# CommonRoad/commonroad-reactive-planner

Measured on AMD Instinct MI355X. Metric: candidate trajectories/sec (sample+cost+collision) per replan, higher is better.
Workload: dtype f64; 1 GPU; cfg3: DEU_Test-1_1_T-1, 31x31x63 grid, N=60, 51 obstacles (49 synthetic, seed 0); mode=draw, horizon_steps=60, n_obstacles=51, parallelism=one GPU, exchange=none

## Files before the change

### commonroad-reactive-planner_amd/csrc/rp_host.hip

```cpp
#include <hip/hip_runtime.h>
#include <hip/hip_ext.h>
#include <sched.h>

#include <algorithm>
#include <atomic>
#include <chrono>
#include <cmath>
#include <cstdio>
#include <cstdlib>
#include <cstring>
#include <mutex>
#include <new>
#include <string>
#include <unordered_map>
#include <vector>

#include "rp_kernels.h"
#include "rp_frontend.h"
#include "rp_corridor.h"
#include "rp_pool.h"

namespace {

constexpr int kBlocksPerCU = 4;
constexpr int kFoldPartials = 256;
constexpr int kFoldThreshold = 8192;
constexpr size_t kAutoMaterializeBytes = 64u << 20;
constexpr size_t kLdsTableLimit = 65536;
constexpr int kChunkMinWavesPerCU = 7;
constexpr int kCostMinPerCU = 832;
constexpr int kSweepMinPerCU = 512;
constexpr int kLazyCap[RP_LAZY_LEVELS] = {1024, 4096, 16384};
constexpr int kLazyOff[RP_LAZY_LEVELS] = {0, 1024, 5120};
constexpr int kLazyListWords = 21504;
constexpr uint32_t kLazyTarget[RP_LAZY_LEVELS] = {128, 1024, 8192};

using ResultBlock = FinalizeOut;

struct Options {
    int lanes = 0;
    int eval_block = 0;
    int cost_kernel = -1;
    int chunk_kernel = -1;
    int lazy = -1;
    int sweep = -1;
    int fused_lon = 1;
    int fused_lon_blocks = -1;
    int auto_materialize = 1;
    int stage_out = 1, row_padding = 1, row_align = 0, tail_split = 1;
    int table_window = 1;
    int fold_threshold = kFoldThreshold;
    int lon_publish = 1, inline_grids = 1, event_bracket = 0, winner_lanes_as_batch = 0, zero_copy = 1, coeff_groups = 1;
    int winner_skip_query = 1;
    int lazy_trace = 0, print_stamps = 0, timing = 0;
    int wait_mode = RP_WAIT_SPIN;
};
struct OptionDesc {
    const char *key;
    int Options::*field;
    const char *env;
    bool env_negates;
    int lo, hi;
};
const OptionDesc kOptionTable[] = {
    {"lanes", &Options::lanes, "RP_AMD_G", false, 0, 64},
    {"eval_block", &Options::eval_block, "RP_AMD_EVAL_BLOCK", false, 0, 256},
    {"cost_kernel", &Options::cost_kernel, "RP_AMD_COST_KERNEL", false, -1, 1},
    {"chunk_kernel", &Options::chunk_kernel, "RP_AMD_CHUNK_KERNEL", false, -1, 1},
    {"lazy", &Options::lazy, "RP_AMD_LAZY", false, -1, 1},
    {"sweep", &Options::sweep, "RP_AMD_SWEEP", false, -1, 1},
    {"fused_lon", &Options::fused_lon, "RP_AMD_NO_FUSED_LON", true, 0, 1},
    {"fused_lon_blocks", &Options::fused_lon_blocks, "RP_AMD_FUSED_LON_BLOCKS", false, -1, 1 << 20},
    {"auto_materialize", &Options::auto_materialize, "RP_AMD_NO_AUTO_MATERIALIZE", true, 0, 1},
    {"stage_out", &Options::stage_out, "RP_AMD_NO_STAGE_OUT", true, 0, 1},
    {"row_padding", &Options::row_padding, "RP_AMD_NO_ROW_PADDING", true, 0, 1},
    {"row_align", &Options::row_align, "RP_AMD_ROW_ALIGN", false, 0, 16},
    {"tail_split", &Options::tail_split, "RP_AMD_NO_TAIL_SPLIT", true, 0, 1},
    {"table_window", &Options::table_window, "RP_AMD_NO_TABLE_WINDOW", true, 0, 1},
    {"fold_threshold", &Options::fold_threshold, "RP_AMD_FOLD_THRESHOLD", false, 1, 1 << 30},
    {"lon_publish", &Options::lon_publish, "RP_AMD_NO_LON_PUBLISH", true, 0, 1},
    {"inline_grids", &Options::inline_grids, "RP_AMD_NO_INLINE_GRIDS", true, 0, 1},
    {"event_bracket", &Options::event_bracket, "RP_AMD_EVENT_BRACKET", false, 0, 1},
    {"winner_lanes_as_batch", &Options::winner_lanes_as_batch, "RP_AMD_WINNER_G_AS_BATCH", false, 0, 1},
    {"winner_skip_query", &Options::winner_skip_query, "RP_AMD_NO_WINNER_SKIP_QUERY", true, 0, 1},
    {"zero_copy", &Options::zero_copy, "RP_AMD_NO_ZERO_COPY", true, 0, 1},
    {"coeff_groups", &Options::coeff_groups, "RP_AMD_NO_COEFF_GROUPS", true, 0, 1},
    {"lazy_trace", &Options::lazy_trace, "RP_AMD_LAZY_TRACE", false, 0, 1},
    {"print_stamps", &Options::print_stamps, "RP_AMD_PRINT_STAMPS", false, 0, 1},
    {"timing", &Options::timing, "RP_AMD_TIMING", false, 0, 1},
    {"wait_mode", &Options::wait_mode, "RP_AMD_WAIT_MODE", false, RP_WAIT_SPIN, RP_WAIT_EVENT},
};
const OptionDesc *find_option(const char *key) {
    if (!key) return nullptr;
    for (const OptionDesc &d : kOptionTable)
        if (std::strcmp(d.key, key) == 0) return &d;
    return nullptr;
}
void options_from_environment(Options &o) {
    for (const OptionDesc &d : kOptionTable) {
        const char *e = d.env ? std::getenv(d.env) : nullptr;
        if (!e) continue;
        const int v = d.env_negates ? 0 : std::atoi(e);
        if (v >= d.lo && v <= d.hi) o.*(d.field) = v;
    }
}

}

struct rp_ctx {
    Options opt;
// ... 18 lines not shown
    std::vector<double> h_sobb, h_tri, h_circ;
    std::vector<int32_t> h_clus_info;
    bool grid_valid = false;
    double grid_ego_r = 0.0;
    int32_t *d_clus_info = nullptr;
    ObsTables obs{};

    char *h_stage = nullptr, *d_stage = nullptr;
    size_t cap_stage = 0;
    std::vector<char> staged;
    bool staged_on_device = false;
    uint32_t *d_status = nullptr;
    double *d_cost = nullptr, *d_user = nullptr;
    size_t cap_status = 0, cap_cost = 0, cap_user = 0;
    double *d_states = nullptr;
    double *d_compact = nullptr;
    size_t cap_compact = 0;
    size_t cap_states = 0;
    double *d_profile = nullptr, *d_profile_one = nullptr;
    size_t cap_profile = 0, cap_profile_one = 0;
    PairHdr *d_pair_hdr = nullptr, *d_pair_hdr_one = nullptr;
    size_t cap_pair_hdr = 0;
    void *d_partials = nullptr;
    int cap_partials = 0;
    unsigned long long *d_sel_scratch = nullptr;
    LazyCtl *d_lazy_ctl = nullptr;
    int32_t *d_lazy_lists = nullptr;
    uint32_t *d_lazy_hist = nullptr;
    double *d_lazy_states = nullptr;
    size_t cap_lazy_states = 0;
    int lazy_skip = 0, lazy_penalty = 0;
    int collision_mode = RP_COLLISION_AUTO;
    int last_kernel = 0;
    int last_lazy = 0;
    double last_best_cost = 0.0;
    int64_t last_best_index = -1;
    double path_us[2] = {0.0, 0.0};
    int path_n[2] = {0, 0};
    int path_since_probe = 0, path_regime = -1;
    bool path_adaptive = false;
    bool time_whole = false;
    std::chrono::steady_clock::time_point plan_t0;
    bool epilogue_dirty = false;
    struct Pending {
        bool active = false, cin = false, skip_eval = false, ticket = false, done = false, time_valid = false, mat = false, coeffs = false;
        unsigned long long seq = 0;
        int grid = 0;
        KArgs ka{};
        std::chrono::steady_clock::time_point tp0, tp1;
    } pending;
    struct LevelState {
        Pending pending;
        std::vector<char> staged;
        bool staged_on_device = false, last_rows_on_device = false;
        int last_G = 0, last_block = 0, last_kernel = 0, last_lazy = 0;
        size_t last_fused_lds = 0;
        int grid_index = 0;
    };
    std::vector<LevelState> chain;
    int chain_total = 0;
    unsigned long long *d_gate = nullptr;
    unsigned long long *d_sweep = nullptr;
    struct ChainInputs {
        rp_params p; rp_cost cost; std::vector<rp_grids> grids; std::vector<std::vector<double>> T, L, D; std::vector<std::vector<int32_t>> tl;
        int want = 0;
    } chain_in;
// ... 116 lines not shown
        if (f && hipExtModuleLaunchKernel(f, (uint32_t)grid * (uint32_t)block, 1, 1, (uint32_t)block, 1, 1, lds, c->stream, nullptr, extra,
                                          c->ev0, c->ev1, 0) == hipSuccess) {
            c->timed_by_launch = true;
            return;
        }
        (void)hipGetLastError();
    }
    if (!f || hipModuleLaunchKernel(f, (unsigned)grid, 1, 1, (unsigned)block, 1, 1, (unsigned)lds, c->stream, nullptr, extra) != hipSuccess) {
        (void)hipGetLastError();
        void *args[] = {const_cast<void *>(args_block)};
        (void)hipLaunchKernel(kernel, dim3(grid), dim3(block), args, lds, c->stream);
    }
}

int collision_level(const KArgs &ka) {
    if (!ka.has_obstacles || (ka.flags & RP_FLAG_SKIP_COLLISION)) return 0;
    return (ka.obs.n_sobb + ka.obs.n_tri + ka.obs.n_circ) > 0 ? 2 : 1;
}

const void *sweep_kernel_fn(bool cin, int coll, bool one_chunk) {
    if (cin) {
        if (coll == 2) return one_chunk ? (const void *)rp_eval_kernel<16, false, true, 2, true, false, false, RP_BLOCK, true> : (const void *)rp_eval_kernel<16, false, true, 2, false, false, false, RP_BLOCK, true>;
        return one_chunk ? (const void *)rp_eval_kernel<16, false, true, 1, true, false, false, RP_BLOCK, true> : (const void *)rp_eval_kernel<16, false, true, 1, false, false, false, RP_BLOCK, true>;
    }
    if (coll == 2) return one_chunk ? (const void *)rp_eval_kernel<16, false, false, 2, true, false, false, RP_BLOCK, true> : (const void *)rp_eval_kernel<16, false, false, 2, false, false, false, RP_BLOCK, true>;
    return one_chunk ? (const void *)rp_eval_kernel<16, false, false, 1, true, false, false, RP_BLOCK, true> : (const void *)rp_eval_kernel<16, false, false, 1, false, false, false, RP_BLOCK, true>;
}

const void *chunk_kernel_fn(bool low, int coll) {
    if (low) return coll == 2 ? (const void *)rp_chunk_kernel<true, 2> : (coll == 1 ? (const void *)rp_chunk_kernel<true, 1> : (const void *)rp_chunk_kernel<true, 0>);
    return coll == 2 ? (const void *)rp_chunk_kernel<false, 2> : (coll == 1 ? (const void *)rp_chunk_kernel<false, 1> : (const void *)rp_chunk_kernel<false, 0>);
}

template <int G, bool MAT, bool CIN, int COLL, bool STAGE>
void launch_eval_tcs(rp_ctx *c, const KArgs &ka, int grid, size_t lds, int block = RP_BLOCK) {
    if constexpr (G == 16 && !STAGE) {
        if (block == 64) {
            if (ka.N + 1 <= G) launch_kargs(c, (const void *)rp_eval_kernel<G, MAT, CIN, COLL, true, false, false, 64>, grid, 64, lds, ka);
            else launch_kargs(c, (const void *)rp_eval_kernel<G, MAT, CIN, COLL, false, false, false, 64>, grid, 64, lds, ka);
            return;
        }
    }
    if (ka.N + 1 <= G) launch_kargs(c, (const void *)rp_eval_kernel<G, MAT, CIN, COLL, true, STAGE, false>, grid, RP_BLOCK, lds, ka);
    else launch_kargs(c, (const void *)rp_eval_kernel<G, MAT, CIN, COLL, false, STAGE, false>, grid, RP_BLOCK, lds, ka);
}

constexpr int kFusedLonG = 16;
constexpr size_t kFusedLonLdsLimit = 61440;
int fused_lon_max_blocks(const rp_ctx *c) {
    if (c->opt.fused_lon_blocks >= 0) return c->opt.fused_lon_blocks;
    return c->num_cus * 4;
}

size_t fused_lon_lds(const rp_ctx *c, const KArgs &ka, int64_t count, int G, bool cin, bool mat, int *pairs) {
    if (count <= 0 || !(G == kFusedLonG || (G == 64 && mat && ka.N + 1 <= 64) || (G == 32 && mat && ka.N + 1 <= 32))) return 0;
    const int gpb = RP_BLOCK / G;
    if ((count + gpb - 1) / gpb > (int64_t)fused_lon_max_blocks(c)) return 0;
    const int P = cin ? gpb : std::min<int64_t>(gpb, ((int64_t)gpb + ka.nD - 2) / ka.nD + 1);
    const size_t slot_bytes = ka.has_obstacles ? (size_t)ka.obs.n_clus * ka.obs.clus_per * RP_SLOT_ROW * sizeof(double) : 0;
    const size_t bytes = (size_t)ka.table_words * sizeof(double) + slot_bytes +
                         (size_t)P * ((size_t)PF_STRIDE * (size_t)(ka.N + 1) * sizeof(double) + sizeof(PairHdr) + sizeof(int) + sizeof(double)) + 16;
    if (bytes > kFusedLonLdsLimit) return 0;
    *pairs = P;
    return (bytes + 15) & ~(size_t)15;
}

template <bool MAT, bool CIN, int COLL>
void launch_eval_fused_c(rp_ctx *c, const KArgs &ka, int grid, size_t lds, int lanes) {
// ... 451 lines not shown
            kl.grids_inline = lon_inline ? 1 : 0;
            kl.publish_grids = lon_publish ? 1 : 0;
            launch_lon(c, kl, cin);
        }
        const bool by_launch = timed && count > 0 && !c->opt.event_bracket;
        const int n_steps = ka.N + 1;
        const int chunk_nb = (n_steps + RP_CHUNK_STEPS - 1) / RP_CHUNK_STEPS;
        const int chunk_G = (chunk_nb >= 2 && chunk_nb <= RP_CHUNK_MAX_BLOCKS) ? chunk_nb : 0;
        const bool lane_kernel_ok = count > 0 && !fused_lds && !cin && !(ka.flags & RP_FLAG_DRAW_ALL) && !ka.single_index && !ka.index_list &&
                                    ka.cost_kind != RP_COST_EXTERNAL;
        const bool cost_rows_ok = (unsigned long long)ka.pair_count * PF_FIELDS * (unsigned long long)(ka.N + 1) * 8ull < (1ull << 32);
        const bool cost_big = count >= (int64_t)c->num_cus * 1024;
        auto lane_kernel_for = [&](int coll) -> int {
            if (!lane_kernel_ok) return 0;
            if (c->opt.chunk_kernel == 1 && chunk_G) return 2;
            if (!cost_rows_ok) return (chunk_G && c->opt.chunk_kernel != 0 && coll == 0) ? 2 : 0;
            if (c->opt.cost_kernel == 1) return 1;
            if (coll > 0) return (c->opt.cost_kernel != 0 && cost_big) ? 1 : 0;
            const int64_t chunk_waves = ((count + RP_CHUNK_BLOCK - 1) / RP_CHUNK_BLOCK) * chunk_G;
            const bool chunk_ok = c->opt.chunk_kernel != 0 && chunk_G && chunk_G <= 4 && chunk_waves >= (int64_t)c->num_cus * kChunkMinWavesPerCU;
            if (c->opt.cost_kernel != 0 && count >= (int64_t)c->num_cus * (chunk_ok ? kCostMinPerCU : (ka.N + 1 <= 64 ? 240 : 448))) return 1;
            return chunk_ok ? 2 : 0;
        };
        auto launch_main_eval = [&](const KArgs &k, bool mat_) -> int {
            c->timed_by_launch = false;
            c->time_next_launch = by_launch;
            if (timed && !by_launch) HIP_TRY(c, hipEventRecord(c->ev0, c->stream));
            const auto te0 = c->timing ? std::chrono::steady_clock::now() : std::chrono::steady_clock::time_point();
            const int coll = collision_level(k);
            const int which = mat_ ? 0 : lane_kernel_for(coll);
            if (which == 1) {
                main_grid = (int)((count + RP_COST_BLOCK - 1) / RP_COST_BLOCK);
                c->last_kernel = RP_KERNEL_COST;
                const void *fn = k.low_vel_mode
                    ? (coll == 2 ? (const void *)rp_cost_kernel<true, 2> : coll == 1 ? (const void *)rp_cost_kernel<true, 1> : (const void *)rp_cost_kernel<true, 0>)
                    : (coll == 2 ? (const void *)rp_cost_kernel<false, 2> : coll == 1 ? (const void *)rp_cost_kernel<false, 1> : (const void *)rp_cost_kernel<false, 0>);
                launch_kargs(c, fn, main_grid, RP_COST_BLOCK, 0, k);
            } else if (which == 2) {
                main_grid = (int)((count + RP_CHUNK_BLOCK - 1) / RP_CHUNK_BLOCK);
                c->last_kernel = RP_KERNEL_CHUNK;
                launch_kargs(c, chunk_kernel_fn(k.low_vel_mode != 0, coll), main_grid, RP_CHUNK_BLOCK * chunk_G, rp_chunk_lds_bytes(chunk_G), k);
            } else {
                main_grid = grid;
                c->last_kernel = RP_KERNEL_EVAL;
                if (fused_lds) launch_eval_fused(c, k, grid, mat_, cin, fused_lds, G);
                else launch_eval(c, k, grid, mat_, cin, G, block);
            }
            if (c->timing) c->t_sum[4] += std::chrono::duration<double, std::micro>(std::chrono::steady_clock::now() - te0).count();
            c->time_next_launch = false;
            if (timed && !by_launch) HIP_TRY(c, hipEventRecord(c->ev1, c->stream));
            time_valid = timed && (!by_launch || c->timed_by_launch);
            return RP_OK;
        };
        bool lazy_possible = count > 0 && !mat && !fused_lds && collision_level(ka) > 0 && !(ka.flags & RP_FLAG_DRAW_ALL) &&
                             ka.cost_kind != RP_COST_EXTERNAL && !ka.single_index && !ka.gate;
        const int lazy_env = c->opt.lazy;
        lazy_possible = lazy_possible && lazy_env != 0 && (c->collision_mode != RP_COLLISION_EAGER || lazy_env == 1);
        const bool always = lazy_env == 1 || (lazy_env == -1 && c->collision_mode == RP_COLLISION_COST_ORDERED);
        bool lazy_try = lazy_possible && (always || (!small && c->lazy_skip == 0));
        if (lazy_possible && !lazy_try && !always && !small && c->lazy_skip > 0) --c->lazy_skip;
        c->path_adaptive = lazy_possible && lazy_env == -1 && !small && c->collision_mode == RP_COLLISION_TIMED;
        if (c->path_adaptive) {
            int lg = 0;
            while ((count >> (lg + 1)) != 0) ++lg;
            const int regime = 2 * lg + (cin ? 1 : 0);
            if (regime != c->path_regime) { c->path_regime = regime; c->path_n[0] = c->path_n[1] = 0; c->path_since_probe = 0; }
            if (lazy_try) {
                if (c->path_n[1] == 0) lazy_try = true;
                else if (c->path_n[0] == 0) lazy_try = c->path_n[1] < 4;
                else {
                    lazy_try = c->path_us[1] <= c->path_us[0];
                    if (++c->path_since_probe >= 64) { lazy_try = !lazy_try; c->path_since_probe = 0; }
                }
            }
        }
        c->last_lazy = 0;
        const bool sweep_first = lazy_try && c->opt.sweep == 1 && !fused_lds;
// ... 322 lines not shown
int rp_last_path(const rp_ctx *c) { return c ? c->last_lazy : 0; }
int rp_last_kernel(const rp_ctx *c) { return c ? c->last_kernel : 0; }

int rp_set_collision_path(rp_ctx *c, int mode) {
    if (!c) return RP_EINVAL;
    if (mode < RP_COLLISION_AUTO || mode > RP_COLLISION_TIMED) return fail(c, RP_EINVAL, "rp_set_collision_path: unknown mode");
    if (mode != c->collision_mode) { c->lazy_skip = c->lazy_penalty = 0; c->path_regime = -1; }
    c->collision_mode = mode;
    return RP_OK;
}

int rp_set_profiling(rp_ctx *c, int enable) {
    if (!c) return RP_EINVAL;
    c->profiling = enable < 0 ? 0 : enable;
    return RP_OK;
}

int rp_set_option(rp_ctx *c, const char *key, int64_t value) {
    if (!c) return RP_EINVAL;
    if (c->pending.active) return fail(c, RP_ESTATE, "rp_set_option: a plan is in flight on this context (rp_plan_wait first)");
    const OptionDesc *d = find_option(key);
    if (!d) return fail(c, RP_EINVAL, std::string("rp_set_option: unknown option '") + (key ? key : "(null)") + "'");
    if (value < d->lo || value > d->hi) return fail(c, RP_EINVAL, std::string("rp_set_option: value out of range for '") + key + "'");
    c->opt.*(d->field) = (int)value;
    c->timing = c->opt.timing != 0;
    c->spin_wait = c->opt.wait_mode != RP_WAIT_EVENT;
    c->lazy_skip = c->lazy_penalty = 0; c->path_regime = -1;
    return RP_OK;
}

int rp_get_option(const rp_ctx *c, const char *key, int64_t *value) {
    if (!c || !value) return RP_EINVAL;
    if (key && std::strcmp(key, "wait_fallbacks") == 0) { *value = c->wait_fallbacks; return RP_OK; }
    const OptionDesc *d = find_option(key);
    if (!d) return RP_EINVAL;
    *value = c->opt.*(d->field);
    return RP_OK;
}

int rp_set_wait_mode(rp_ctx *c, int mode) { return rp_set_option(c, "wait_mode", mode); }
int rp_get_wait_mode(const rp_ctx *c) { return c ? c->opt.wait_mode : RP_WAIT_SPIN; }

int rp_set_reference(rp_ctx *c, int32_t n, const double *ref_pos, const double *ref_theta, const double *ref_curv,
                     const double *ref_curv_d, const double *ref_x, const double *ref_y, double proj_domain_d_limit) {
    if (!c) return RP_EINVAL;
    if (c->pending.active) return fail(c, RP_ESTATE, "rp_set_reference: a plan is in flight on this context (rp_plan_wait first)");
    if (n < 2 || !ref_pos || !ref_theta || !ref_curv || !ref_curv_d || !ref_x || !ref_y)
        return fail(c, RP_EINVAL, "rp_set_reference: need n >= 2 and six non-null tables");
    for (int i = 0; i + 1 < n; ++i)
        if (!(ref_pos[i + 1] > ref_pos[i])) return fail(c, RP_EINVAL, "rp_set_reference: ref_pos must be strictly increasing");
    HIP_TRY(c, hipSetDevice(c->device));
    std::vector<double> t((size_t)TB_ROWS * (size_t)n);
    std::memcpy(&t[(size_t)TB_POS * n], ref_pos, sizeof(double) * n);
    std::memcpy(&t[(size_t)TB_THETA * n], ref_theta, sizeof(double) * n);
    std::memcpy(&t[(size_t)TB_CURV * n], ref_curv, sizeof(double) * n);
    std::memcpy(&t[(size_t)TB_CURV_D * n], ref_curv_d, sizeof(double) * n);
    std::memcpy(&t[(size_t)TB_X * n], ref_x, sizeof(double) * n);
    std::memcpy(&t[(size_t)TB_Y * n], ref_y, sizeof(double) * n);
    double *tx = &t[(size_t)TB_TX * n], *ty = &t[(size_t)TB_TY * n];
    std::vector<double> ux(n - 1), uy(n - 1);
    for (int i = 0; i + 1 < n; ++i) {
        double ex = ref_x[i + 1] - ref_x[i], ey = ref_y[i + 1] - ref_y[i];
        double ln = std::sqrt(ex * ex + ey * ey);
        if (!(ln > 0.0)) return fail(c, RP_EINVAL, "rp_set_reference: duplicate polyline vertices");
        ux[i] = ex / ln; uy[i] = ey / ln;
    }
// ... 1256 lines not shown
```

### commonroad-reactive-planner_amd/csrc/rp_kernels.h

```cpp
#pragma once

#include "rp_device.h"

#define RP_BLOCK 256
#ifndef RP_COPY_OUT_STORE
#define RP_COPY_OUT_STORE(p, v)                                                                                   \
    __builtin_nontemporal_store(*reinterpret_cast<const __attribute__((ext_vector_type(2))) double *>(&(v)),        \
                                reinterpret_cast<__attribute__((ext_vector_type(2))) double *>(p))
#endif
#ifndef RP_WAVES_PER_SIMD
#define RP_WAVES_PER_SIMD 3
#endif

struct KArgs {
    double dt;
    int32_t N, factor, time_step0, low_vel_mode, lon_mode;
    uint32_t constraint_mask, flags;
    double x0_lon[3], x0_lat[3], x0_orientation;
    double wheelbase, wb_rear_axle, half_length, half_width, ego_radius;
    double a_max, v_switch, v_delta_max, kappa_max;
    double c_yaw;
    double c_kdot;
    int32_t cost_kind, has_speed, has_s, partials_cap;
    double w_a, desired_speed, desired_d, desired_s;
// ... 832 lines not shown
            for (int l = 0; l < RP_LAZY_LEVELS; ++l) total[l] += (unsigned int)__popcll(__ballot(lvl[u] == l));
        unsigned int at[RP_LAZY_LEVELS] = {0, 0, 0};
#pragma unroll
        for (int l = 0; l < RP_LAZY_LEVELS; ++l)
            if (total[l] && lane == 0) at[l] = atomicAdd(&a.ctl->count[l], total[l]);
#pragma unroll
        for (int l = 0; l < RP_LAZY_LEVELS; ++l) at[l] = (unsigned int)__builtin_amdgcn_readfirstlane((int)at[l]);
#pragma unroll
        for (int u = 0; u < kUnroll; ++u) {
            const int i = base0 + u * RP_GATHER_THREADS + lane;
#pragma unroll
            for (int l = 0; l < RP_LAZY_LEVELS; ++l) {
                const unsigned long long bm = __ballot(lvl[u] == l);
                const unsigned int pos = at[l] + (unsigned int)__popcll(bm & lt_mask);
                if (lvl[u] == l && pos < (unsigned int)a.cap[l]) a.lists[a.off[l] + (int)pos] = (int32_t)(a.cand_begin + i);
                at[l] += (unsigned int)__popcll(bm);
            }
        }
    }
}

__device__ __forceinline__ double frenet_kterm(double k_r_d, double d, double k_r, double dp) { return __builtin_fma(k_r_d, d, k_r * dp); }
__device__ __forceinline__ double frenet_kappa(double dpp, double kterm, double tanT, double cosT, double q, double k_r) {
    return __builtin_fma(k_r, q, (__builtin_fma(kterm, tanT, dpp) * cosT) * (q * q));
}
__device__ __forceinline__ double heading_cos(double cos_ref, double sin_ref, double cosT, double sinT) { return __builtin_fma(cos_ref, cosT, -(sin_ref * sinT)); }
__device__ __forceinline__ double heading_sin(double cos_ref, double sin_ref, double cosT, double sinT) { return __builtin_fma(sin_ref, cosT, cos_ref * sinT); }
__device__ __forceinline__ double frenet_acc(double sdd, double f, double sd, double secT, double oneKrD, double tanT, double kappa, double k_r,
                                             double kterm) {
    return __builtin_fma(sdd, f, (sd * sd * secT) * __builtin_fma(oneKrD * tanT, __builtin_fma(kappa, f, -k_r), -kterm));
}


template <class KA>
__device__ __forceinline__ double cost_terms(const KA &a, int i, int N, int mid, double acc, double v, double s, double d, double th_cl) {
    double e, cst;
    e = a.w_a * acc; cst = e * e;
    e = 0.25 * (a.desired_d - d); cst = __builtin_fma(e, e, cst);
    e = 0.25 * fabs(th_cl); cst = __builtin_fma(e, e, cst);
    if (a.has_speed) { e = 5.0 * (v - a.desired_speed); cst = __builtin_fma(e, e, cst); }
    if (a.has_s) { e = 0.25 * (a.desired_s - s); cst = __builtin_fma(e, e, cst); }
    if (i == N) {
        e = 20.0 * (a.desired_d - d); cst = __builtin_fma(e, e, cst);
        e = 5.0 * fabs(th_cl); cst = __builtin_fma(e, e, cst);
        if (a.has_speed) { e = v - a.desired_speed; cst += 50.0 * (e * e); }
        if (a.has_s) { e = 20.0 * (a.desired_s - s); cst = __builtin_fma(e, e, cst); }
    }
    if (i == mid && a.has_speed) { e = v - a.desired_speed; cst += 100.0 * (e * e); }
    return cst;
}

template <class KA>
__device__ __forceinline__ uint32_t constraint_reason(const KA &a, uint32_t cm, double v, double acc, double kappa, double dth, double kdot) {
    uint32_t reason = RP_REASON_NONE;
    const double a_max = a.a_max, v_switch = a.v_switch, kappa_max = a.kappa_max;
    const double wk = a.wheelbase * kappa;
    const bool bad_yaw = fabs(rint(dth * a.c_yaw)) > kappa_max * v * 1e5;
    const bool bad_kd = fabs(kdot) > a.c_kdot * __builtin_fma(wk, wk, 1.0);
    const bool fast = v > v_switch;
    const double acc_l = fast ? acc * v : acc, acc_r = fast ? a_max * v_switch : a_max;
    const bool bad_acc = !((-a_max <= acc) & (acc_l <= acc_r));
    const bool bad_v = v < -RP_EPS, bad_k = fabs(kappa) > kappa_max;
    reason = (((cm & RP_CHECK_ACCELERATION) != 0) & bad_acc) ? RP_REASON_ACCELERATION : reason;
    reason = (((cm & RP_CHECK_KAPPA_DOT) != 0) & bad_kd) ? RP_REASON_KAPPA_DOT : reason;
    reason = (((cm & RP_CHECK_YAW_RATE) != 0) & bad_yaw) ? RP_REASON_YAW_RATE : reason;
    reason = (((cm & RP_CHECK_KAPPA) != 0) & bad_k) ? RP_REASON_KAPPA : reason;
// ... 513 lines not shown
template <bool COEFFS_IN>
__device__ __forceinline__ void fetch_lateral(const KArgs &a, int64_t gidx, CandIn &ci, int64_t hdr_pair0) {
    int64_t pair;
    if (COEFFS_IN) {
        const double *pt = a.lat_coeffs + 6 * gidx;
#pragma unroll
        for (int k = 0; k < 6; ++k) ci.v[k] = pt[k];
        pair = pair_index<true>(a, gidx);
    } else {
        const uint32_t g32 = (uint32_t)gidx, nd = (uint32_t)a.nD;
        const uint32_t p32 = g32 / nd;
        pair = p32;
        ci.v[0] = grid_base(a)[a.nT + a.nL + (int)(g32 - p32 * nd)];
    }
    ci.pair_slot = pair - hdr_pair0;
}

__device__ __forceinline__ void fetch_header(const PairHdr *hdrs, CandIn &ci) {
    const PairHdr h = hdrs[ci.pair_slot];
    ci.lat_T = h.lat_T;
    ci.s0 = h.s0;
    ci.pre_reason = h.pre_reason;
    ci.L = h.L;
}

template <bool COEFFS_IN>
__device__ __forceinline__ CandIn fetch_candidate(const KArgs &a, int64_t gidx, const PairHdr *hdrs, int64_t hdr_pair0) {
    CandIn ci;
    fetch_lateral<COEFFS_IN>(a, gidx, ci, hdr_pair0);
    fetch_header(hdrs, ci);
    return ci;
}

template <int G, bool MAT, bool COEFFS_IN, int COLL, bool ONE_CHUNK, bool STAGE_OUT, bool LON_FUSED, int BLOCK = RP_BLOCK, bool SWEEP = false>
__global__ __launch_bounds__(BLOCK, RP_WAVES_PER_SIMD) void rp_eval_kernel(const KArgsG ag) {
    static_assert(!SWEEP || (G == 16 && !MAT && COLL != 0 && !STAGE_OUT && !LON_FUSED && BLOCK == RP_BLOCK), "the sweep's variant");
    const KArgs &a = ag.k;
    extern __shared__ double lds_out[];
    static_assert(!(LON_FUSED && STAGE_OUT), "the single-launch variant stores state rows directly");
    constexpr bool RP_WT = LON_FUSED;
    constexpr bool RP_NT = MAT && !LON_FUSED && !STAGE_OUT;
    touch_kernargs<10>();

    const int tid = threadIdx.x;
    RP_STAMP(0);
    RP_TL(0);
    const int lane = tid & 63;
    const int gl = lane & (G - 1);
    const int gbase = lane & ~(G - 1);
    static_assert(BLOCK == RP_BLOCK || (!LON_FUSED && !STAGE_OUT), "smaller workgroups: plain two-kernel variants only");
    constexpr int GPB = BLOCK / G;
    constexpr int GPW = 64 / G;
    constexpr int PFN = COLL ? PF_FIELDS : PF_COS_REF;
    const int wave_in_block = tid >> 6;
    const int group_in_wave = gbase / G;
    const int grp = tid / G;

    if (level_gate_closed(a.gate, a.gate_seq, a.gate_level)) return;
    if (a.single_index && *a.single_index < 0) {
        if (a.host_seq && a.ticket_if_none && tid == 0) __hip_atomic_store(a.host_seq, a.seq_value, __ATOMIC_RELEASE, __HIP_MEMORY_SCOPE_SYSTEM);
        return;
    }
    const int64_t wave_first = ((int64_t)blockIdx.x * GPB) + (int64_t)wave_in_block * GPW;
    int64_t count_ = a.single_index ? 1 : a.count;
    if (!LON_FUSED && a.index_list) {
        const uint32_t lc = *a.list_count;
        count_ = (int64_t)(lc < (uint32_t)a.list_cap ? lc : (uint32_t)a.list_cap);
        if ((int64_t)blockIdx.x * GPB >= count_) {
            if (a.partials) {
// ... 286 lines not shown
    }
    RP_STAMP(1);

    typedef const KArgs __attribute__((address_space(4))) *kargs_cptr;
    kargs_cptr ap_late = (LON_FUSED || MAT) ? (kargs_cptr)__builtin_amdgcn_kernarg_segment_ptr() : (kargs_cptr)&a;
    if (LON_FUSED) asm volatile("" : "+s"(ap_late));
    const KArgs __attribute__((address_space(4))) &al = *ap_late;
    const int N = al.N, n = N + 1;
    const int nchunks = ONE_CHUNK ? 1 : (n + G - 1) / G;
    const double dt = al.dt;
    const bool draw = (al.flags & RP_FLAG_DRAW_ALL) != 0;
    const bool low = al.low_vel_mode != 0;
    const uint32_t cm = al.constraint_mask;
    const int mid = n / 2;
    double *const gs_poly = sh_grp[grp].poly;
    double *const gs_last = sh_grp[grp].last;

    auto eval_cost_terms = [&](int i, double acc, double v, double s, double d, double th_cl) -> double {
        double e, cst;
        e = al.w_a * acc; cst = e * e;
        e = 0.25 * (al.desired_d - d); cst = __builtin_fma(e, e, cst);
        e = 0.25 * fabs(th_cl); cst = __builtin_fma(e, e, cst);
        if (al.has_speed) { e = 5.0 * (v - al.desired_speed); cst = __builtin_fma(e, e, cst); }
        if (al.has_s) { e = 0.25 * (al.desired_s - s); cst = __builtin_fma(e, e, cst); }
        if (i == N) {
            e = 20.0 * (al.desired_d - d); cst = __builtin_fma(e, e, cst);
            e = 5.0 * fabs(th_cl); cst = __builtin_fma(e, e, cst);
            if (al.has_speed) { e = v - al.desired_speed; cst += 50.0 * (e * e); }
            if (al.has_s) { e = 20.0 * (al.desired_s - s); cst = __builtin_fma(e, e, cst); }
        }
        if (i == mid && al.has_speed) { e = v - al.desired_speed; cst += 100.0 * (e * e); }
        return cst;
    };

    if (wave_first < count) {
        const int64_t w0 = wave_first;
        const int64_t slot = w0 + group_in_wave;
        const bool valid = slot < count && sweep_need;
        const int64_t gidx = al.single_index ? *al.single_index
                             : ((!LON_FUSED && al.index_list) ? (int64_t)al.index_list[valid ? slot : w0] : al.cand_begin + (valid ? slot : w0));

        const int L = cin.L;
        const double s0 = cin.s0;
        const uint32_t pre_reason = (uint32_t)cin.pre_reason;
        const int32_t pair_slot_ = (int32_t)(pair_index<COEFFS_IN>(al, gidx) - pair0);
        const int32_t pair_w = __builtin_amdgcn_readfirstlane(pair_slot_);
        const uint32_t n8p = (uint32_t)n * 8u;
        const char *const pbase = reinterpret_cast<const char *>(prof_base + ((size_t)pair_w * PF_FIELDS) * (size_t)n);
        const uint32_t poff8 = (uint32_t)(pair_slot_ - pair_w) * PF_FIELDS * n8p;
        ProfStep pf = pf0;
        if (!LON_FUSED) {
            Poly lat;
            if (COEFFS_IN) lat = {cin.v[0], cin.v[1], cin.v[2], cin.v[3], cin.v[4], cin.v[5]};
            else lat = quintic_coeffs(al.x0_lat[0], al.x0_lat[1], al.x0_lat[2], cin.v[0], 0.0, 0.0, cin.lat_T);
            if (gl == 0) park_poly(gs_poly, lat);
        }
        RP_STAMP(2);

        int fail_step = -1, ood_step = -1;
        uint32_t fail_reason = RP_REASON_NONE;
        bool collide = false;
        double cost_acc = 0.0;

        bool alive = valid && pre_reason == RP_REASON_NONE;
        if (__ballot(alive) != 0) {
            double theta_carry = al.x0_orientation;
            double kappa_carry = 0.0;
            double cumx = 0.0, cumy = 0.0;
            const bool store_ok = MAT && valid && pre_reason == RP_REASON_NONE;
            const int ns = (MAT && !STAGE_OUT) ? al.row_stride : n;
            constexpr bool SPLIT_OK = MAT && !STAGE_OUT && !LON_FUSED && G == 16;
            const int tail_m = SPLIT_OK ? al.tail_split : 0;
            const uint32_t cand8 = (uint32_t)state_block_doubles(ns, tail_m) * 8u;
            char *const obase = !MAT ? nullptr
                                : (STAGE_OUT ? reinterpret_cast<char *>(lds_out + (size_t)(wave_in_block * GPW) * RP_N_ARRAYS * (size_t)n)
                                             : reinterpret_cast<char *>(al.states) + (size_t)w0 * (size_t)cand8);
            const uint32_t n8 = (uint32_t)ns * 8u;
            const uint32_t lane_off8 = (uint32_t)group_in_wave * (STAGE_OUT ? RP_N_ARRAYS * n8 : cand8);
            constexpr bool ROW_MULV = LON_FUSED;
            constexpr bool LATE_STORE = MAT && !STAGE_OUT;
            uint32_t n8v = n8;
            auto row_at = [&](uint32_t off8, int row) -> double * {
                return reinterpret_cast<double *>(obase + (size_t)(ROW_MULV ? __umul24((uint32_t)row, n8v) + off8 : off8 + (uint32_t)row * n8));
            };

#pragma nounroll
            for (int c = 0; c < nchunks; ++c) {
                const int base = c * G;
                const int i = base + gl;
                const bool live = i <= N;
                const bool act = i < L;
                if (ROW_MULV) asm volatile("" : "+v"(n8v));

                if (!ONE_CHUNK && c > 0) {
                    if (LON_FUSED) pf = load_profile_item<PFN>(prof_base + ((size_t)pair_slot_ * (size_t)n + (size_t)(live ? i : N)) * PF_STRIDE);
                    else pf = load_profile<PFN, G == 16>(pbase, poff8 + (uint32_t)(live ? i : N) * 8u, n8p);
                }
                double s = pf.f[PF_S], sd = pf.f[PF_SD], sdd = pf.f[PF_SDD];
                const double inv_sd = pf.f[PF_INV_SD], th_ref = pf.f[PF_TH_REF];
                const double k_r = pf.f[PF_KR], k_r_d = pf.f[PF_KRD];
                const double px = pf.f[PF_PX], py = pf.f[PF_PY], nx = pf.f[PF_NX], ny = pf.f[PF_NY];
                const bool s_in_dom = pf.f[PF_INDOM] != 0.0;

                constexpr bool SKIP_EXTENDED = !(MAT && COLL == 0);
                double d = 0.0, dd = 0.0, ddd = 0.0, th_cl = 0.0, th_gl = 0.0, cos_gl = 1.0, sin_gl = 0.0;
                double kappa = 0.0, v = 0.0, acc = 0.0, kdot = 0.0, x = 0.0, y = 0.0;
                uint64_t near_sta_cell = 0;
                if (!SKIP_EXTENDED || __any(act)) {
                    const double t = (double)i * dt;
                    const double tau = low ? s - s0 : t;
                    d = poly_pos(gs_poly, tau); dd = poly_vel(gs_poly, tau); ddd = poly_acc(gs_poly, tau);
                    if (fabs(dd) < RP_EPS) dd = 0.0;
                    if (!LATE_STORE && store_ok && act) {
                        const uint32_t off8 = lane_off8 + (uint32_t)i * 8u;
                        st_row<RP_WT, RP_NT>(row_at(off8, RP_S), s);
                        st_row<RP_WT, RP_NT>(row_at(off8, RP_S_DOT), sd);
                        st_row<RP_WT, RP_NT>(row_at(off8, RP_S_DDOT), sdd);
                        st_row<RP_WT, RP_NT>(row_at(off8, RP_D), d);
                        st_row<RP_WT, RP_NT>(row_at(off8, RP_D_DOT), dd);
                        st_row<RP_WT, RP_NT>(row_at(off8, RP_D_DDOT), ddd);
                    }
                    RP_STAMP(3);

                    const bool moving = inv_sd > 0.0;
                    double dp, dpp;
                    lateral_derivs(low, dd, ddd, inv_sd, sdd, dp, dpp);

                    const bool use_atan = moving || low;
                    double cosT, secT, tanT;
                    atan_angles(dp, th_ref, th_cl, th_gl, cosT, secT, tanT);
                    if (__any(act && !use_atan)) {
                        const uint64_t mv = group_ballot<G>(use_atan && act, gbase);
                        const uint64_t below = mv & ((1ull << gl) - 1ull);
                        const int src = below ? 63 - __clzll(below) : 0;
                        const double th_from = group_bcast<G>(th_gl, src);
                        if (!use_atan) {
                            th_gl = below ? th_from : theta_carry;
// ... 15 lines not shown
                    RP_STAMP(6);

                    uint32_t reason = constraint_reason(al, cm, v, acc, kappa, dth, kdot);
                    reason = act ? reason : RP_REASON_NONE;
                    if (__any(reason != RP_REASON_NONE)) {
                        const uint64_t fm = group_ballot<G>(reason != RP_REASON_NONE, gbase);
                        const int fl = fm ? __ffsll((unsigned long long)fm) - 1 : 0;
                        const uint32_t r_first = (uint32_t)__shfl((int)reason, fl, G);
                        if (fm && fail_step < 0) { fail_step = base + fl; fail_reason = r_first; }
                        if (!draw && fail_step >= 0) alive = false;
                        if (__ballot(alive) == 0) break;
                    }
                    RP_STAMP(7);

                    const bool in_dom = s_in_dom && fabs(d) <= al.proj_d_limit;
                    x = px + d * nx; y = py + d * ny;
                    if (__any(act && !in_dom) || ood_step >= 0) {
                        const uint64_t om = group_ballot<G>(act && !in_dom, gbase);
                        if (om && ood_step < 0) ood_step = base + __ffsll((unsigned long long)om) - 1;
                        if (ood_step >= 0 && i >= ood_step) { x = 0.0; y = 0.0; }
                    }
                    if (act) {
                        if (!LATE_STORE && store_ok) {
                            const uint32_t off8 = lane_off8 + (uint32_t)i * 8u;
                            st_row<RP_WT, RP_NT>(row_at(off8, RP_X), x);
                            st_row<RP_WT, RP_NT>(row_at(off8, RP_Y), y);
                            st_row<RP_WT, RP_NT>(row_at(off8, RP_THETA), th_gl);
                            st_row<RP_WT, RP_NT>(row_at(off8, RP_V), v);
                            st_row<RP_WT, RP_NT>(row_at(off8, RP_A), acc);
                            st_row<RP_WT, RP_NT>(row_at(off8, RP_KAPPA), kappa);
                            st_row<RP_WT, RP_NT>(row_at(off8, RP_KAPPA_DOT), kdot);
                            st_row<RP_WT, RP_NT>(row_at(off8, RP_THETA_CL), th_cl);
                        }
                        cost_acc += eval_cost_terms(i, acc, v, s, d, th_cl);
                    }
                    if (COLL == 2 && live && alive && fail_step < 0 && ood_step < 0 && !collide && act)
                        near_sta_cell = static_grid_mask(al.obs.grid, al.obs.gx0, al.obs.gy0, al.obs.ginv, al.obs.gnx, al.obs.gny,
                                                         x + al.wb_rear_axle * cos_gl, y + al.wb_rear_axle * sin_gl);
                }
                const bool cell_wanted = COLL == 2 && live && alive && fail_step < 0 && ood_step < 0 && !collide;
                RP_STAMP(8);

                const int ll = L - 1 - base;
                const bool take = (ll >= 0 && ll < G);
                if (__any(take && L < n)) {
                    if (!COLL) rp_sincos(th_gl, &sin_gl, &cos_gl);
                    if (take && gl == ll) {
                        double *o = gs_last;
                        o[0] = x; o[1] = y; o[2] = th_gl; o[3] = v; o[4] = acc; o[5] = kappa; o[6] = kdot;
                        o[7] = s; o[8] = d; o[9] = th_cl; o[10] = sd; o[11] = sdd; o[12] = dd; o[13] = ddd;
                        o[14] = cos_gl; o[15] = sin_gl;
                    }
                }
                if (!ONE_CHUNK && c + 1 < nchunks) {
                    theta_carry = group_bcast<G>(th_gl, G - 1);
                    kappa_carry = group_bcast<G>(kappa, G - 1);
                }
                if (__any(live && !act)) {
                    double termx = 0.0, termy = 0.0;
                    const double *o = gs_last;
                    const double tk = (double)(i - L + 1) * dt;
                    double vt = 0.0;
                    if (!act) {
                        vt = o[3] + tk * o[4];
                        vt = vt * (vt >= 0.0 ? 1.0 : 0.0);
                        termx = dt * vt * o[14];
                        termy = dt * vt * o[15];
                    }
                    const double scx = group_scan<G>(termx) + cumx, scy = group_scan<G>(termy) + cumy;
                    if (!act) {
                        x = o[0] + scx;
                        y = o[1] + scy;
                        th_gl = o[2];
                        cos_gl = o[14];
                        sin_gl = o[15];
                        const double sv = o[10] + tk * 0.0;
                        const double e_sd = sv * (sv >= 0.0 ? 1.0 : 0.0);
                        const double e_dd = o[12] + tk * 0.0;
                        const double e_s = o[7] + tk * o[10];
                        const double e_d = o[8] + tk * o[12];
                        if (live) cost_acc += eval_cost_terms(i, o[4], vt, e_s, e_d, o[9]);
                        if (LATE_STORE) {
                            v = vt; acc = o[4]; kappa = o[5]; kdot = o[6];
                            s = e_s; d = e_d; th_cl = o[9];
                            sd = e_sd; sdd = o[11]; dd = e_dd; ddd = o[13];
                        } else if (store_ok && live) {
                            {
                                const uint32_t off8 = lane_off8 + (uint32_t)i * 8u;
                                st_row<RP_WT, RP_NT>(row_at(off8, RP_X), x);
                                st_row<RP_WT, RP_NT>(row_at(off8, RP_Y), y);
                                st_row<RP_WT, RP_NT>(row_at(off8, RP_THETA), th_gl);
                                st_row<RP_WT, RP_NT>(row_at(off8, RP_V), vt);
                                st_row<RP_WT, RP_NT>(row_at(off8, RP_A), o[4]);
                                st_row<RP_WT, RP_NT>(row_at(off8, RP_KAPPA), o[5]);
                                st_row<RP_WT, RP_NT>(row_at(off8, RP_KAPPA_DOT), o[6]);
                                st_row<RP_WT, RP_NT>(row_at(off8, RP_S), e_s);
                                st_row<RP_WT, RP_NT>(row_at(off8, RP_D), e_d);
                                st_row<RP_WT, RP_NT>(row_at(off8, RP_THETA_CL), o[9]);
                                st_row<RP_WT, RP_NT>(row_at(off8, RP_S_DOT), e_sd);
                                st_row<RP_WT, RP_NT>(row_at(off8, RP_S_DDOT), o[11]);
                                st_row<RP_WT, RP_NT>(row_at(off8, RP_D_DOT), e_dd);
                                st_row<RP_WT, RP_NT>(row_at(off8, RP_D_DDOT), o[13]);
                            }
                        }
                    }
                    if (!ONE_CHUNK && c + 1 < nchunks) {
                        cumx = group_bcast<G>(scx, G - 1);
                        cumy = group_bcast<G>(scy, G - 1);
                    }
                }
                if (COLL == 2) {
                    if (cell_wanted && !act)
                        near_sta_cell = static_grid_mask(al.obs.grid, al.obs.gx0, al.obs.gy0, al.obs.ginv, al.obs.gnx, al.obs.gny,
                                                         x + al.wb_rear_axle * cos_gl, y + al.wb_rear_axle * sin_gl);
                    uint32_t c_lo = (uint32_t)near_sta_cell, c_hi = (uint32_t)(near_sta_cell >> 32);
                    asm volatile("" : "+v"(c_lo), "+v"(c_hi));
                    near_sta_cell = ((uint64_t)c_hi << 32) | c_lo;
                }
                if (SPLIT_OK && tail_m > 0 && base >= tail_m) {
                    if (store_ok) {
                        char *const tbase = obase + (size_t)(lane_off8 + (uint32_t)(RP_N_ARRAYS * tail_m) * 8u + (uint32_t)gl * 8u);
                        const bool lo = gl < 8;
                        auto pair_store = [&](int q, double r0, double r1) {
                            const double up = dpp_f64<DPP_ROW_SHR8, 0xf>(r1);
                            st_row<RP_WT, RP_NT>(reinterpret_cast<double *>(tbase + q * 128), lo ? r0 : up);
                        };
                        pair_store(0, x, y); pair_store(1, th_gl, v); pair_store(2, acc, kappa); pair_store(3, kdot, s);
                        pair_store(4, d, th_cl); pair_store(5, sd, sdd); pair_store(6, dd, ddd);
                    }
                } else
                if (LATE_STORE && store_ok && i < ns) {
                    const uint32_t off8 = lane_off8 + (uint32_t)i * 8u;
                    st_row<RP_WT, RP_NT>(row_at(off8, RP_X), x);
                    st_row<RP_WT, RP_NT>(row_at(off8, RP_Y), y);
                    st_row<RP_WT, RP_NT>(row_at(off8, RP_THETA), th_gl);
                    st_row<RP_WT, RP_NT>(row_at(off8, RP_V), v);
                    st_row<RP_WT, RP_NT>(row_at(off8, RP_A), acc);
                    st_row<RP_WT, RP_NT>(row_at(off8, RP_KAPPA), kappa);
                    st_row<RP_WT, RP_NT>(row_at(off8, RP_KAPPA_DOT), kdot);
                    st_row<RP_WT, RP_NT>(row_at(off8, RP_S), s);
                    st_row<RP_WT, RP_NT>(row_at(off8, RP_D), d);
                    st_row<RP_WT, RP_NT>(row_at(off8, RP_THETA_CL), th_cl);
                    st_row<RP_WT, RP_NT>(row_at(off8, RP_S_DOT), sd);
                    st_row<RP_WT, RP_NT>(row_at(off8, RP_S_DDOT), sdd);
                    st_row<RP_WT, RP_NT>(row_at(off8, RP_D_DOT), dd);
                    st_row<RP_WT, RP_NT>(row_at(off8, RP_D_DDOT), ddd);
                }
                RP_STAMP(9);

                if (COLL) {
                    const bool want = live && alive && fail_step < 0 && ood_step < 0 && !collide;
                    bool hit = false;
                    constexpr bool masked = !COEFFS_IN;
                    const uint64_t near_dyn = double_as_mask(pf.f[PF_NEAR]);
                    const double ego_cx = x + al.wb_rear_axle * cos_gl, ego_cy = y + al.wb_rear_axle * sin_gl;
                    const uint64_t near_sta = want ? near_sta_cell : 0;
                    const bool ask = want && ((!masked && al.obs.n_dyn > 0) || (near_dyn | near_sta) != 0);
                    RP_STAMP(44);
#ifdef RP_WALK_COUNT
                    if (a.debug && !a.single_index && blockIdx.x == RP_STAMP_BLOCK && threadIdx.x == RP_STAMP_THREAD) rp_walk_dbg = a.debug + 40;
#endif
// ... 721 lines not shown
```

Baseline: 455.4 million candidates/s.

## Add fixed 64-stride eval kernel variant with deferred, freshly fetched cost params

Adds a ROW64 template specialization of the eval kernel, used when the row stride is 64, tail split is off and the horizon fits in 64 steps. With a compile-time stride, state-row addresses are computed from a single mid-row base with constant offsets. Cost evaluation and static-grid lookup move out of the inner loop to after the extension, with cost parameters reloaded from a scalar pointer. The intent is to cut address arithmetic and register pressure in the materializing path, at the cost of another kernel instantiation and a different cost-accumulation point.

```diff
diff --git a/commonroad-reactive-planner_amd/csrc/rp_host.hip b/commonroad-reactive-planner_amd/csrc/rp_host.hip
--- a/commonroad-reactive-planner_amd/csrc/rp_host.hip
+++ b/commonroad-reactive-planner_amd/csrc/rp_host.hip
@@ -48,6 +48,7 @@
     int fused_lon_blocks = -1;
     int auto_materialize = 1;
     int stage_out = 1, row_padding = 1, row_align = 0, tail_split = 1;
+    int fixed_stride = 1;
     int table_window = 1;
     int fold_threshold = kFoldThreshold;
     int lon_publish = 1, inline_grids = 1, event_bracket = 0, winner_lanes_as_batch = 0, zero_copy = 1, coeff_groups = 1;
@@ -76,6 +77,7 @@
     {"row_padding", &Options::row_padding, "RP_AMD_NO_ROW_PADDING", true, 0, 1},
     {"row_align", &Options::row_align, "RP_AMD_ROW_ALIGN", false, 0, 16},
     {"tail_split", &Options::tail_split, "RP_AMD_NO_TAIL_SPLIT", true, 0, 1},
+    {"fixed_stride", &Options::fixed_stride, "RP_AMD_NO_FIXED_STRIDE", true, 0, 1},
     {"table_window", &Options::table_window, "RP_AMD_NO_TABLE_WINDOW", true, 0, 1},
     {"fold_threshold", &Options::fold_threshold, "RP_AMD_FOLD_THRESHOLD", false, 1, 1 << 30},
     {"lon_publish", &Options::lon_publish, "RP_AMD_NO_LON_PUBLISH", true, 0, 1},
@@ -160,6 +162,7 @@
     int lazy_skip = 0, lazy_penalty = 0;
     int collision_mode = RP_COLLISION_AUTO;
     int last_kernel = 0;
+    int last_fixed_stride = 0;
     int last_lazy = 0;
     double last_best_cost = 0.0;
     int64_t last_best_index = -1;
@@ -342,8 +345,19 @@
     return coll == 2 ? (const void *)rp_chunk_kernel<false, 2> : (coll == 1 ? (const void *)rp_chunk_kernel<false, 1> : (const void *)rp_chunk_kernel<false, 0>);
 }
 
+inline bool fixed_stride_applies(const rp_ctx *c, const KArgs &ka) {
+    return ka.row_stride == RP_ROW64 && ka.tail_split == 0 && ka.N + 1 > 16 && ka.N + 1 <= RP_ROW64 && c->opt.fixed_stride != 0;
+}
+
 template <int G, bool MAT, bool CIN, int COLL, bool STAGE>
 void launch_eval_tcs(rp_ctx *c, const KArgs &ka, int grid, size_t lds, int block = RP_BLOCK) {
+    if constexpr (G == 16 && MAT && !STAGE) {
+        if (fixed_stride_applies(c, ka)) {
+            if (block == 64) launch_kargs(c, (const void *)rp_eval_kernel<G, MAT, CIN, COLL, false, false, false, 64, false, true>, grid, 64, lds, ka);
+            else launch_kargs(c, (const void *)rp_eval_kernel<G, MAT, CIN, COLL, false, false, false, RP_BLOCK, false, true>, grid, RP_BLOCK, lds, ka);
+            return;
+        }
+    }
     if constexpr (G == 16 && !STAGE) {
         if (block == 64) {
             if (ka.N + 1 <= G) launch_kargs(c, (const void *)rp_eval_kernel<G, MAT, CIN, COLL, true, false, false, 64>, grid, 64, lds, ka);
@@ -861,6 +875,7 @@
             if (which == 1) {
                 main_grid = (int)((count + RP_COST_BLOCK - 1) / RP_COST_BLOCK);
                 c->last_kernel = RP_KERNEL_COST;
+                c->last_fixed_stride = 0;
                 const void *fn = k.low_vel_mode
                     ? (coll == 2 ? (const void *)rp_cost_kernel<true, 2> : coll == 1 ? (const void *)rp_cost_kernel<true, 1> : (const void *)rp_cost_kernel<true, 0>)
                     : (coll == 2 ? (const void *)rp_cost_kernel<false, 2> : coll == 1 ? (const void *)rp_cost_kernel<false, 1> : (const void *)rp_cost_kernel<false, 0>);
@@ -868,10 +883,12 @@
             } else if (which == 2) {
                 main_grid = (int)((count + RP_CHUNK_BLOCK - 1) / RP_CHUNK_BLOCK);
                 c->last_kernel = RP_KERNEL_CHUNK;
+                c->last_fixed_stride = 0;
                 launch_kargs(c, chunk_kernel_fn(k.low_vel_mode != 0, coll), main_grid, RP_CHUNK_BLOCK * chunk_G, rp_chunk_lds_bytes(chunk_G), k);
             } else {
                 main_grid = grid;
                 c->last_kernel = RP_KERNEL_EVAL;
+                c->last_fixed_stride = !fused_lds && mat_ && G == 16 && fixed_stride_applies(c, k);
                 if (fused_lds) launch_eval_fused(c, k, grid, mat_, cin, fused_lds, G);
                 else launch_eval(c, k, grid, mat_, cin, G, block);
             }
@@ -1260,6 +1277,7 @@
 int rp_get_option(const rp_ctx *c, const char *key, int64_t *value) {
     if (!c || !value) return RP_EINVAL;
     if (key && std::strcmp(key, "wait_fallbacks") == 0) { *value = c->wait_fallbacks; return RP_OK; }
+    if (key && std::strcmp(key, "last_fixed_stride") == 0) { *value = c->last_fixed_stride; return RP_OK; }
     const OptionDesc *d = find_option(key);
     if (!d) return RP_EINVAL;
     *value = c->opt.*(d->field);
diff --git a/commonroad-reactive-planner_amd/csrc/rp_kernels.h b/commonroad-reactive-planner_amd/csrc/rp_kernels.h
--- a/commonroad-reactive-planner_amd/csrc/rp_kernels.h
+++ b/commonroad-reactive-planner_amd/csrc/rp_kernels.h
@@ -888,6 +888,7 @@
 }
 
 
+struct CostParams { double w_a, desired_speed, desired_d, desired_s; int32_t has_speed, has_s; };
 template <class KA>
 __device__ __forceinline__ double cost_terms(const KA &a, int i, int N, int mid, double acc, double v, double s, double d, double th_cl) {
     double e, cst;
@@ -1467,9 +1468,12 @@
     return ci;
 }
 
-template <int G, bool MAT, bool COEFFS_IN, int COLL, bool ONE_CHUNK, bool STAGE_OUT, bool LON_FUSED, int BLOCK = RP_BLOCK, bool SWEEP = false>
+#define RP_ROW64 64
+template <int G, bool MAT, bool COEFFS_IN, int COLL, bool ONE_CHUNK, bool STAGE_OUT, bool LON_FUSED, int BLOCK = RP_BLOCK, bool SWEEP = false,
+          bool ROW64 = false>
 __global__ __launch_bounds__(BLOCK, RP_WAVES_PER_SIMD) void rp_eval_kernel(const KArgsG ag) {
     static_assert(!SWEEP || (G == 16 && !MAT && COLL != 0 && !STAGE_OUT && !LON_FUSED && BLOCK == RP_BLOCK), "the sweep's variant");
+    static_assert(!ROW64 || (G == 16 && MAT && !ONE_CHUNK && !STAGE_OUT && !LON_FUSED && !SWEEP), "the fixed-stride variant");
     const KArgs &a = ag.k;
     extern __shared__ double lds_out[];
     static_assert(!(LON_FUSED && STAGE_OUT), "the single-launch variant stores state rows directly");
@@ -1822,6 +1826,22 @@
         if (i == mid && al.has_speed) { e = v - al.desired_speed; cst += 100.0 * (e * e); }
         return cst;
     };
+    auto fetched_cost_terms = [&](const CostParams &cp, int i, double acc, double v, double s, double d, double th_cl) -> double {
+        double e, cst;
+        e = cp.w_a * acc; cst = e * e;
+        e = 0.25 * (cp.desired_d - d); cst = __builtin_fma(e, e, cst);
+        e = 0.25 * fabs(th_cl); cst = __builtin_fma(e, e, cst);
+        if (cp.has_speed) { asm volatile(""); e = 5.0 * (v - cp.desired_speed); cst = __builtin_fma(e, e, cst); }
+        if (cp.has_s) { asm volatile(""); e = 0.25 * (cp.desired_s - s); cst = __builtin_fma(e, e, cst); }
+        if (i == N) {
+            e = 20.0 * (cp.desired_d - d); cst = __builtin_fma(e, e, cst);
+            e = 5.0 * fabs(th_cl); cst = __builtin_fma(e, e, cst);
+            if (cp.has_speed) { asm volatile(""); e = v - cp.desired_speed; cst += 50.0 * (e * e); }
+            if (cp.has_s) { asm volatile(""); e = 20.0 * (cp.desired_s - s); cst = __builtin_fma(e, e, cst); }
+        }
+        if (i == mid && cp.has_speed) { asm volatile(""); e = v - cp.desired_speed; cst += 100.0 * (e * e); }
+        return cst;
+    };
 
     if (wave_first < count) {
         const int64_t w0 = wave_first;
@@ -1858,8 +1878,8 @@
             double kappa_carry = 0.0;
             double cumx = 0.0, cumy = 0.0;
             const bool store_ok = MAT && valid && pre_reason == RP_REASON_NONE;
-            const int ns = (MAT && !STAGE_OUT) ? al.row_stride : n;
-            constexpr bool SPLIT_OK = MAT && !STAGE_OUT && !LON_FUSED && G == 16;
+            const int ns = ROW64 ? RP_ROW64 : ((MAT && !STAGE_OUT) ? al.row_stride : n);
+            constexpr bool SPLIT_OK = MAT && !STAGE_OUT && !LON_FUSED && G == 16 && !ROW64;
             const int tail_m = SPLIT_OK ? al.tail_split : 0;
             const uint32_t cand8 = (uint32_t)state_block_doubles(ns, tail_m) * 8u;
             char *const obase = !MAT ? nullptr
@@ -1893,6 +1913,7 @@
                 const bool s_in_dom = pf.f[PF_INDOM] != 0.0;
 
                 constexpr bool SKIP_EXTENDED = !(MAT && COLL == 0);
+                constexpr bool LEAN = ROW64;
                 double d = 0.0, dd = 0.0, ddd = 0.0, th_cl = 0.0, th_gl = 0.0, cos_gl = 1.0, sin_gl = 0.0;
                 double kappa = 0.0, v = 0.0, acc = 0.0, kdot = 0.0, x = 0.0, y = 0.0;
                 uint64_t near_sta_cell = 0;
@@ -1974,9 +1995,9 @@
                             st_row<RP_WT, RP_NT>(row_at(off8, RP_KAPPA_DOT), kdot);
                             st_row<RP_WT, RP_NT>(row_at(off8, RP_THETA_CL), th_cl);
                         }
-                        cost_acc += eval_cost_terms(i, acc, v, s, d, th_cl);
+                        if (!LEAN) cost_acc += eval_cost_terms(i, acc, v, s, d, th_cl);
                     }
-                    if (COLL == 2 && live && alive && fail_step < 0 && ood_step < 0 && !collide && act)
+                    if (!LEAN && COLL == 2 && live && alive && fail_step < 0 && ood_step < 0 && !collide && act)
                         near_sta_cell = static_grid_mask(al.obs.grid, al.obs.gx0, al.obs.gy0, al.obs.ginv, al.obs.gnx, al.obs.gny,
                                                          x + al.wb_rear_axle * cos_gl, y + al.wb_rear_axle * sin_gl);
                 }
@@ -2021,7 +2042,7 @@
                         const double e_dd = o[12] + tk * 0.0;
                         const double e_s = o[7] + tk * o[10];
                         const double e_d = o[8] + tk * o[12];
-                        if (live) cost_acc += eval_cost_terms(i, o[4], vt, e_s, e_d, o[9]);
+                        if (!LEAN && live) cost_acc += eval_cost_terms(i, o[4], vt, e_s, e_d, o[9]);
                         if (LATE_STORE) {
                             v = vt; acc = o[4]; kappa = o[5]; kdot = o[6];
                             s = e_s; d = e_d; th_cl = o[9];
@@ -2051,8 +2072,15 @@
                         cumy = group_bcast<G>(scy, G - 1);
                     }
                 }
+                if (LEAN) {
+                    static_assert(!LEAN || LATE_STORE, "the lanes' row values are the extended state behind the extension");
+                    kargs_cptr ac = ap_late;
+                    asm volatile("" : "+s"(ac));
+                    const CostParams cp = {ac->w_a, ac->desired_speed, ac->desired_d, ac->desired_s, ac->has_speed, ac->has_s};
+                    if (live) cost_acc += fetched_cost_terms(cp, i, acc, v, s, d, th_cl);
+                }
                 if (COLL == 2) {
-                    if (cell_wanted && !act)
+                    if (cell_wanted && (LEAN || !act))
                         near_sta_cell = static_grid_mask(al.obs.grid, al.obs.gx0, al.obs.gy0, al.obs.ginv, al.obs.gnx, al.obs.gny,
                                                          x + al.wb_rear_axle * cos_gl, y + al.wb_rear_axle * sin_gl);
                     uint32_t c_lo = (uint32_t)near_sta_cell, c_hi = (uint32_t)(near_sta_cell >> 32);
@@ -2069,6 +2097,28 @@
                         };
                         pair_store(0, x, y); pair_store(1, th_gl, v); pair_store(2, acc, kappa); pair_store(3, kdot, s);
                         pair_store(4, d, th_cl); pair_store(5, sd, sdd); pair_store(6, dd, ddd);
+                    }
+                } else
+                if (ROW64) {
+                    if (store_ok) {
+                        char *mid_row = obase + (size_t)(lane_off8 + (uint32_t)i * 8u + 7u * (RP_ROW64 * 8u));
+                        asm volatile("" : "+v"(mid_row));
+                        typedef double __attribute__((address_space(1))) *grow;
+                        auto row64 = [&](int row) -> double * { return (double *)(grow)(uintptr_t)(mid_row + (row - 7) * (RP_ROW64 * 8)); };
+                        st_row<RP_WT, RP_NT>(row64(RP_X), x);
+                        st_row<RP_WT, RP_NT>(row64(RP_Y), y);
+                        st_row<RP_WT, RP_NT>(row64(RP_THETA), th_gl);
+                        st_row<RP_WT, RP_NT>(row64(RP_V), v);
+                        st_row<RP_WT, RP_NT>(row64(RP_A), acc);
+                        st_row<RP_WT, RP_NT>(row64(RP_KAPPA), kappa);
+                        st_row<RP_WT, RP_NT>(row64(RP_KAPPA_DOT), kdot);
+                        st_row<RP_WT, RP_NT>(row64(RP_S), s);
+                        st_row<RP_WT, RP_NT>(row64(RP_D), d);
+                        st_row<RP_WT, RP_NT>(row64(RP_THETA_CL), th_cl);
+                        st_row<RP_WT, RP_NT>(row64(RP_S_DOT), sd);
+                        st_row<RP_WT, RP_NT>(row64(RP_S_DDOT), sdd);
+                        st_row<RP_WT, RP_NT>(row64(RP_D_DOT), dd);
+                        st_row<RP_WT, RP_NT>(row64(RP_D_DDOT), ddd);
                     }
                 } else
                 if (LATE_STORE && store_ok && i < ns) {
```

Measured after the change: 464.7 million candidates/s (median of 6 runs). +2.0%, better.
